# ouguangjun/Leg-KILO

Measured on NVIDIA H100. Metric: LiDAR point-iterations/sec through the ESKF point-to-plane update, higher is better.
Workload: dtype f64

## Files before the change

leg-kilo_b200/csrc/lk_api.cu:

```cuda
#include <cmath>
#include <cstdio>
#include <chrono>
#include <cstring>
#include <mutex>
#include <string>
#include <vector>

#include "lk_host.h"
#include "lk_kernels.h"
#include "lk_mapdev.h"

namespace lk {
int decode_pointcloud2_device(const uint8_t* h_data, uint32_t n, const lk_pc2_layout& L, float blind, int filter_num,
                              double time_scale, float* h_pts_out, float* h_intensity_out, uint32_t* n_out, cudaStream_t s,
                              std::string& err);
int preprocess_scan_device(const float* h_pts_in, uint32_t n, float leaf, float* h_pts_out, uint32_t* n_out,
                           uint32_t* h_bucket_offsets, float* h_bucket_curv, uint32_t* n_buckets, cudaStream_t s,
                           std::string& err);
size_t leg_kinematics_scratch_bytes(uint32_t n);
int leg_kinematics_device(const lk_leg_cfg& cfg, const lk_leg_state* h_in, uint32_t n, int redundancy,
                          lk_leg_track* track, lk_kinimu_meas* h_out, uint32_t* n_out, void* scratch, cudaStream_t s,
                          std::string& err);
}

// ... 24 lines not shown
          initsL(chunksL + align256(n_chunksL * sizeof(ChunkDesc))),
          bytes(initsL + align256(n_initsL * sizeof(StepInit))) {}
};

struct OutBlock {
    size_t x = 0, P = 0, clk = 0, n_eff = 0, status = 0, bytes = 0;
    OutBlock() = default;
    explicit OutBlock(int batch)
        : P(align256((size_t)batch * sizeof(lk_state))),
          clk(P + align256((size_t)batch * 900 * 8)),
          n_eff(clk + align256((size_t)batch * sizeof(lk_stream_clock))),
          status(n_eff + align256((size_t)batch * 4)),
          bytes(status + 256) {}
};

}

struct lk_context {
    int device = 0;
    cudaStream_t stream = nullptr;
    std::string err;
    lk_eskf_cfg ec;
    lk_map_cfg mc;
    Globals g;

    MapDevHost map;
    double last_slide_position[3] = {0.0, 0.0, 0.0};

    int batch = 0;
    uint64_t total_pts = 0;
    uint32_t total_chunks = 0, n_steps = 0, max_chunk_pts = 0;
    std::vector<ChunkDesc> h_chunks, h_chunksL;
    InBlock in;
    OutBlock out;
    DevBuf pts, world, sc, step, partial, ticket, fb_list, fb_cnt;
    DevBuf small_in, small_out, fx, fP, fQ, fclk;
    PinnedBuf h_small_in, h_small_out;
    DevView chunks, stepinit, x_in, P_in, clk_in, Q, x, P, clk, n_eff, status;
    DevBuf dbg_ok, dbg_h, dbg_z, dbg_R, dbg_key, tmp, trace, bar;
    DevBuf ins_pts, ins_root, ins_pend, ins_touched, ins_counters, ins_list;
    uint64_t ins_pend_nodes = 0;
    DevBuf mi_pts, mi_small, mi_ipts, mi_root, mi_touched, mi_counters, mi_list;
    PinnedBuf h_mi;
    int trace_on = 0;
    uint32_t trace_seq = 0;
    int lane_cache = 1;
    int use_fused = 1;
    FusedInline inl;
    DevBuf ll;
    uint32_t ll_epoch = 1;
    bool prev_fused = false;
    uint32_t fused_launches = 0, fused_launches_since_check = 0;
    int direct_io = 1, inline_in = 1, coop_launch = 0, pdl = 1, n_sms = 132, slim_p = 1;
    int fast_insert = 1;
    int fused_insert = 0;
    int debug_records = 0;
    bool direct = false, direct_ran = false, inline_ok = false;
    const float4* direct_pts = nullptr;
    float4* direct_world = nullptr;
    double hprof[8] = {0, 0, 0, 0, 0, 0, 0, 0};
    DevBuf Qc;
    DevBuf leg_scratch;
    std::vector<double> Q_shadow;

    cudaEvent_t ev0 = nullptr, ev1 = nullptr;
    std::vector<cudaEvent_t> kev;
    float last_total_ms = 0, last_residual_ms = 0;
    uint32_t last_launches = 0, last_residual_launches = 0;
    uint32_t acc_launches = 0, acc_residual_launches = 0;
    size_t nev = 0;
    int kernel_timing = 1;
    std::vector<StepInit> h_inits;
    std::vector<uint32_t> h_scan_pts;
    std::vector<uint32_t> h_scan_chunks;
    std::vector<StepInit> h_initsL;
    DevView chunksL, stepinitL;
    uint32_t total_chunksL = 0;

    ~lk_context() {
        for (cudaEvent_t e : kev) cudaEventDestroy(e);
        if (ev0) cudaEventDestroy(ev0);
        if (ev1) cudaEventDestroy(ev1);
        if (stream) cudaStreamDestroy(stream);
    }
};

namespace {

int fail(lk_handle h, int code, const std::string& msg) {
    if (h) h->err = msg;
    else g_create_error = msg;
    return code;
}

struct FusedGate {
    std::mutex m;
    cudaStream_t last = nullptr;
    cudaEvent_t ev = nullptr;
};
FusedGate& fused_gate(int device) {
    static FusedGate gates[64];
    return gates[(device >= 0 && device < 64) ? device : 0];
}

void enter(lk_handle h) {
    cudaSetDevice(h->device);
// ... 181 lines not shown
int lk_init_process_cov(const lk_eskf_cfg* c, double* Q) {
    if (!c || !Q) return LK_ERR_INVALID_ARG;
    for (int i = 0; i < 900; ++i) Q[i] = 0.0;
    const double d[7] = {c->vel_process_cov,     c->acc_bias_process_cov, c->gyr_bias_process_cov, c->imu_acc_process_cov,
                         c->imu_gyr_process_cov, c->kin_bias_process_cov, c->contact_process_cov};
    const int at[7] = {6, 9, 12, 18, 21, 24, 27};
    for (int b = 0; b < 7; ++b)
        for (int k = 0; k < 3; ++k) Q[(at[b] + k) * 30 + at[b] + k] = d[b];
    return LK_OK;
}

int lk_state_default(lk_state* x) {
    if (!x) return LK_ERR_INVALID_ARG;
    std::memset(x, 0, sizeof(*x));
    x->rot[0] = x->rot[4] = x->rot[8] = 1.0;
    x->grav[2] = -9.81;
    return LK_OK;
}

int lk_leg_track_default(lk_leg_track* t) {
    if (!t) return LK_ERR_INVALID_ARG;
    for (int k = 0; k < 4; ++k) t->in_contact[k] = 1;
    t->last_acc_z = 0.0f;
    t->last_gyr_z = 0.0f;
    return LK_OK;
}

int lk_host_alloc(void** p, size_t bytes) {
    if (!p) return LK_ERR_INVALID_ARG;
    cudaError_t e = cudaHostAlloc(p, bytes, cudaHostAllocDefault);
    if (e != cudaSuccess) {
        cudaGetLastError();
        return LK_ERR_OUT_OF_MEMORY;
    }
    return LK_OK;
}

int lk_host_free(void* p) {
    if (p) cudaFreeHost(p);
    return LK_OK;
}

int lk_set_param(lk_handle h, const char* name, double value) {
    if (!h || !name) return LK_ERR_INVALID_ARG;
    using IntKnob = int lk_context::*;
    static const struct {
        const char* name;
        IntKnob knob;
    } knobs[] = {{"kernel_timing", &lk_context::kernel_timing}, {"fused", &lk_context::use_fused},
                 {"lane_cache", &lk_context::lane_cache},       {"fast_insert", &lk_context::fast_insert},
                 {"fused_insert", &lk_context::fused_insert},   {"coop_launch", &lk_context::coop_launch},
                 {"pdl", &lk_context::pdl},                     {"slim_p", &lk_context::slim_p},
                 {"direct_io", &lk_context::direct_io},         {"inline_in", &lk_context::inline_in},
                 {"debug_records", &lk_context::debug_records}};
    for (const auto& k : knobs)
        if (!std::strcmp(name, k.name)) {
            h->*k.knob = (int)value;
            return LK_OK;
        }
    if (!std::strcmp(name, "trace")) {
        h->trace_on = (int)value;
        if (h->trace_on) {
            enter(h);
            LK_CUDA(h->err, h->trace.ensure((size_t)(1 << 16) * 8 * 8));
            LK_CUDA(h->err, cudaMemset(h->trace.p, 0, (size_t)(1 << 16) * 8 * 8));
        }
        h->trace_seq = 0;
        return LK_OK;
    }
    return fail(h, LK_ERR_INVALID_ARG, std::string("unknown parameter ") + name);
}

int lk_debug_read(lk_handle h, int what, void* dst, size_t bytes) {
    if (!h || !dst) return LK_ERR_INVALID_ARG;
    if (what == 3) {
        std::memcpy(dst, h->hprof, std::min(bytes, sizeof(h->hprof)));
        std::memset(h->hprof, 0, sizeof(h->hprof));
        return LK_OK;
    }
    enter(h);
    DevBuf* b = what == 0 ? &h->partial : (what == 1 ? &h->sc : &h->trace);
    if (what == 2) h->trace_seq = 0;
    if (bytes > b->cap) bytes = b->cap;
    LK_CUDA(h->err, cudaMemcpy(dst, b->p, bytes, cudaMemcpyDeviceToHost));
    return LK_OK;
}

int lk_sync(lk_handle h) {
    if (!h) return LK_ERR_INVALID_ARG;
    enter(h);
    LK_CUDA(h->err, cudaStreamSynchronize(h->stream));
    return check_stall(h);
}


int lk_map_reserve(lk_handle h, uint64_t max_roots, uint64_t max_nodes, uint64_t max_points) {
    if (!h) return LK_ERR_INVALID_ARG;
    h->map.reserve_roots = max_roots;
    h->map.reserve_nodes = max_nodes;
    h->map.reserve_points = max_points;
    return LK_OK;
}

int lk_map_upload(lk_handle h, const void* blob, size_t bytes) {
    if (!h || !blob) return fail(h, LK_ERR_INVALID_ARG, "null argument");
    enter(h);
    return map_upload_blob(h->map, h->g, blob, bytes, h->stream, h->err);
// ... 289 lines not shown
    LK_CUDA(h->err, cudaGetLastError());
    {
        const int rc = check_stall(h);
        if (rc) return rc;
    }
    LK_CUDA(h->err, cudaEventElapsedTime(&h->last_total_ms, h->ev0, h->ev1));
    float rms = 0;
    for (size_t i = 0; i + 1 < h->nev; i += 2) {
        float ms = 0;
        cudaEventElapsedTime(&ms, h->kev[i], h->kev[i + 1]);
        rms += ms;
    }
    h->last_residual_ms = rms;
    h->last_launches = h->acc_launches;
    h->last_residual_launches = h->acc_residual_launches;
    if (total_ms) *total_ms = h->last_total_ms;
    if (residual_kernel_ms) *residual_kernel_ms = rms;
    if (n_kernel_launches) *n_kernel_launches = h->last_launches;
    if (n_residual_launches) *n_residual_launches = h->last_residual_launches;
    return LK_OK;
}

namespace {
struct MeasQueue {
    const lk_imu_meas* d_imu = nullptr;
    const lk_kinimu_meas* d_kin = nullptr;
    const double* stamps = nullptr;
    uint32_t n = 0;
    double gravity = 9.81, acc_norm = 1.0;
};
}

static FusedArgs fused_args(lk_handle h, uint32_t first, int iters, bool insert, const MeasQueue* mq) {
    FusedArgs fa;
    std::memset(&fa, 0, sizeof(fa));
    fa.pts = h->direct ? h->direct_pts : h->pts.as<float4>();
    fa.world = h->direct ? h->direct_world : h->world.as<float4>();
    fa.inits = h->stepinit.as<StepInit>();
    fa.batch = h->batch;
    fa.n_steps = h->n_steps;
    fa.scan = first;
    fa.x_in = h->x_in.as<double>();
    fa.P_in = h->P_in.as<double>();
    fa.clk_in = h->clk_in.as<lk_stream_clock>();
    fa.Q = h->Q.as<double>();
    fa.x = h->x.as<double>();
    fa.P = h->P.as<double>();
    fa.clk = h->clk.as<lk_stream_clock>();
    fa.n_eff = h->n_eff.as<uint32_t>();
    fa.status = h->status.as<uint32_t>();
    fa.ll.chunk_rows = h->ll.as<ulonglong2>();
    fa.ll.group_rows = h->ll.as<ulonglong2>() + (size_t)2 * LL_MAX_CHUNKS * LL_ROW;
    fa.ll.stall = reinterpret_cast<uint32_t*>((char*)h->ll.p + LL_ROWS_BYTES);
    fa.epoch = h->ll_epoch;
    fa.iters = iters;
    fa.lane_cache = h->lane_cache;
    {
        const lk_stream_clock* ck = reinterpret_cast<const lk_stream_clock*>((const char*)h->h_small_in.p + h->in.clk) + first;
        const StepInit& in0 = h->h_inits[first];
        fa.slim_p = h->slim_p && h->n_steps == 1 && !mq && in0.active && in0.t_bucket == ck->last_predict_time &&
                    in0.t_bucket == ck->last_update_time;
    }
    const MapDev md = h->map.dev();
    fa.mv.slots = md.slots;
    fa.mv.hash_mask = md.hash_mask;
    fa.mv.nodes = md.nodes;
    fa.mv.hot = md.hot;
    if (mq) {
        fa.imu = mq->d_imu;
        fa.kin = mq->d_kin;
        fa.n_meas = mq->n;
        fa.gravity = mq->gravity;
        fa.acc_norm = mq->acc_norm;
    }
    fa.ecfg = h->ec;
    fa.trace = h->trace_on ? h->trace.as<unsigned long long>() + (size_t)(h->trace_seq++ % TRACE_AREAS) * TRACE_AREA : nullptr;
    fa.g = h->g;
    if (insert) {
        fa.insert = 1;
        fa.md = md;
        fa.ipts = reinterpret_cast<DevPoint*>(h->ins_pts.p);
        fa.iroot = h->ins_root.as<int>();
        fa.pend = h->ins_pend.as<int>();
        fa.touched = h->ins_touched.as<uint32_t>();
        fa.ins_counters = h->ins_counters.as<uint32_t>() + 2;
    }
    return fa;
}

static int run_fused(lk_handle h, uint32_t first, int iters, bool insert, const MeasQueue* mq, bool timed) {
    cudaStream_t s = h->stream;
    const uint32_t grid = insert ? (uint32_t)fused_max_blocks(h->device) : h->h_scan_chunks[first];
    FusedInline* inl = nullptr;
    if (h->inline_ok) {
        const char* hs = (const char*)h->h_small_in.p;
        inl = &h->inl;
        std::memcpy(inl->x, hs + h->in.x, sizeof(inl->x));
        std::memcpy(inl->P, hs + h->in.P, sizeof(inl->P));
        std::memcpy(inl->clk, hs + h->in.clk, sizeof(inl->clk));
        std::memcpy(inl->steps, h->h_inits.data(), h->h_inits.size() * sizeof(StepInit));
    }
    const uint32_t need = h->n_steps * ((uint32_t)iters + 2u) + 1u;
    if (h->ll_epoch > 0xE0000000u || need > 0x10000000u) {
        if (need > 0x10000000u) return fail(h, LK_ERR_INVALID_ARG, "steps x iters too large for one launch");
        LK_CUDA(h->err, cudaMemsetAsync(h->ll.p, 0, LL_BYTES, s));
        h->ll_epoch = 1;
        h->prev_fused = false;
    }
    const FusedArgs fa = fused_args(h, first, iters, insert, mq);
    h->ll_epoch += need;
    if (insert) h->prev_fused = false;
    if (timed) { cudaEventRecord(kev_get(h, h->nev++), s); h->prev_fused = false; }
    const int mode = h->coop_launch ? FUSED_LAUNCH_COOPERATIVE : ((h->pdl && h->prev_fused) ? FUSED_LAUNCH_PDL : FUSED_LAUNCH_PLAIN);
    {
        FusedGate& gate = fused_gate(h->device);
        std::lock_guard<std::mutex> lock(gate.m);
        if (gate.last && gate.last != s) {
            if (!gate.ev) LK_CUDA(h->err, cudaEventCreateWithFlags(&gate.ev, cudaEventDisableTiming));
            LK_CUDA(h->err, cudaEventRecord(gate.ev, gate.last));
            LK_CUDA(h->err, cudaStreamWaitEvent(s, gate.ev, 0));
        }
        gate.last = s;
        LK_CUDA(h->err, launch_scan_fused(fa, inl, grid, s, mode));
    }
    h->prev_fused = true;
    ++h->fused_launches_since_check;
    if (timed) { cudaEventRecord(kev_get(h, h->nev++), s); h->prev_fused = false; }
    ++h->acc_launches;
    ++h->acc_residual_launches;
    h->direct_ran = h->direct;
    return LK_OK;
}

static int run_kernels(lk_handle h, uint32_t first, uint32_t count, int iters, bool update_map, const MeasQueue* mq,
                       bool timed) {
    cudaStream_t s = h->stream;
    const int batch = h->batch;
    const bool big = count >= 2 && !h->h_initsL.empty();
    const std::vector<StepInit>& tin = big ? h->h_initsL : h->h_inits;
    const ChunkDesc* d_chunks = big ? h->chunksL.as<ChunkDesc>() : h->chunks.as<ChunkDesc>();
    const StepInit* d_inits = big ? h->stepinitL.as<StepInit>() : h->stepinit.as<StepInit>();
    uint32_t small_parity = 0;
    uint32_t mi = 0;
    if (mq) {
        LK_CUDA(h->err, cudaMemcpyAsync(h->x.as<lk_state>() + first, h->x_in.as<lk_state>() + first, sizeof(lk_state), cudaMemcpyDeviceToDevice, s));
        LK_CUDA(h->err, cudaMemcpyAsync(h->P.as<double>() + (size_t)first * 900, h->P_in.as<double>() + (size_t)first * 900, 900 * 8, cudaMemcpyDeviceToDevice, s));
        LK_CUDA(h->err, cudaMemcpyAsync(h->clk.as<lk_stream_clock>() + first, h->clk_in.as<lk_stream_clock>() + first, sizeof(lk_stream_clock), cudaMemcpyDeviceToDevice, s));
        LK_CUDA(h->err, cudaMemsetAsync(h->n_eff.as<uint32_t>() + first, 0, 4, s));
    }
    for (uint32_t k = 0; k < h->n_steps; ++k) {
        const StepInit* hin = tin.data() + (size_t)k * batch;
        uint32_t c0 = hin[first].chunk_begin, c1 = hin[first + count - 1].chunk_end;
        uint32_t m_obs0 = mi, m_obs1 = mi;
        if (mq && hin[first].active) {
            while (m_obs1 < mq->n && mq->stamps[m_obs1] < hin[first].t_bucket) ++m_obs1;
            mi = m_obs1;
        }
        const PredictArgs pa = predict_args(h, d_inits + (size_t)k * batch, (k == 0 && !mq) ? 1 : 0, first, count);
        if (mq && count == 1 && hin[first].active)
            launch_obs_predict_prepare(pa, mq->d_imu ? mq->d_imu + m_obs0 : nullptr, mq->d_kin ? mq->d_kin + m_obs0 : nullptr,
                                       m_obs1 - m_obs0, h->ec, mq->gravity, mq->acc_norm, s);
        else
// ... 504 lines not shown
```

leg-kilo_b200/csrc/lk_fused.cu:

```cuda
#include "lk_insert.cuh"
#include "lk_kernels.h"
#include "lk_obs.cuh"
#include "lk_pass.cuh"
#include "lk_predict.cuh"
#include "lk_solve.cuh"

namespace lk {

namespace {

#define FT(slot) do { if (a.trace && threadIdx.x == 0 && (slot) < 32) a.trace[(size_t)blockIdx.x * 32 + (slot)] = gtime(); } while (0)
#define FTI(slot) do { if (it_global < 3) FT(slot); } while (0)
#define FTS(slot) do { if (a.trace && blockIdx.x == 0 && threadIdx.x == 0 && k < 64) a.trace[(size_t)gridDim.x * 32 + (size_t)k * 8 + (slot)] = gtime(); } while (0)
#ifndef LK_HOP_TRACE
#define LK_HOP_TRACE 0
#endif
#define FT_HOPS() ((LK_HOP_TRACE && a.trace && it_global < 3) \
                       ? a.trace + (size_t)gridDim.x * 32 + 64 * 8 + (size_t)blockIdx.x * 16 + it_global * LL_HOP_SLOTS : nullptr)

constexpr int BLOCK = FB;
constexpr int WARPS = BLOCK / 32;

struct PredictScratch {
    double F[900];
// ... 30 lines not shown
    for (uint32_t t = blockIdx.x * (uint32_t)WARPS + (uint32_t)warp; t < n_touched; t += gridDim.x * (uint32_t)WARPS)
        warp_insert_root_scan(md, si->g, wt, __ldcg(&touched[t]), iroot, ipts, n_bucket, pend, lane);
}

static_assert(sizeof(PredictScratch) <= sizeof(((PassSmem<BLOCK, true>*)0)->tile) &&
                  sizeof(PredictScratch) <= sizeof(((PassSmem<BLOCK, false>*)0)->tile),
              "predict scratch must not reach the mbarriers");
static_assert(sizeof(FusedSmemIns) <= 227 * 1024, "one block per SM");
static_assert(sizeof(FusedSmem) + 1024 <= 132 * 1024, "the batch-of-one kernel's stack frames must fit in L1");

int carveout_percent(size_t smem, int dev) {
    int per_sm = 0, per_block = 0;
    cudaDeviceGetAttribute(&per_sm, cudaDevAttrMaxSharedMemoryPerMultiprocessor, dev);
    cudaDeviceGetAttribute(&per_block, cudaDevAttrReservedSharedMemoryPerBlock, dev);
    if (per_sm <= 0) return 100;
    const size_t need = smem + (size_t)per_block;
    const int pct = (int)((need * 100 + (size_t)per_sm - 1) / (size_t)per_sm);
    return pct < 100 ? pct : 100;
}

template <class SM>
__device__ __noinline__ void fused_predict(SM* sm, const double* Q, double dtc, double dt) {
    if (dtc != 0.0) {
        build_F(sm->u.pr.F, sm->f.x, dtc);
        cov_predict(sm->f.P, sm->u.pr.F, sm->u.pr.T, sm->u.pr.Ps, Q, dtc);
    }
    if (dt != 0.0) {
        if (threadIdx.x == 0) state_predict(sm->f.x, dt);
    }
    fence_proxy_async();
    __syncthreads();
}

template <class SM>
__device__ __noinline__ void fused_drain_queue(SM* sm, const FusedArgs& a, uint32_t& mi, double t_bucket) {
    bool drained = false;
    while (mi < a.n_meas) {
        const double ts = a.imu ? a.imu[mi].stamp : a.kin[mi].stamp;
        if (!(ts < t_bucket)) break;
        block_predict_to(&sm->f, sm->clk, ts, sm->u.pr.F, sm->u.pr.T, sm->u.pr.Ps, a.Q);
        if (a.imu) block_obs_imu<BLOCK>(&sm->f, &sm->u.pr.obs, a.imu + mi, &a.ecfg, a.gravity, a.acc_norm);
        else block_obs_kinimu<BLOCK>(&sm->f, &sm->u.pr.obs, a.kin + mi, &a.ecfg, a.gravity, a.acc_norm);
        if (threadIdx.x == 0) sm->clk[1] = ts;
        __syncthreads();
        ++mi;
        drained = true;
    }
    if (drained) {
        fence_proxy_async();
        __syncthreads();
    }
}

template <bool INL> struct InlineSel { typedef FusedInline type; };
template <> struct InlineSel<false> { typedef FusedNoInline type; };

__device__ __forceinline__ void grid_sync(const FusedArgs& a, uint32_t& sync_idx) {
    __threadfence();
    __syncthreads();
    if (threadIdx.x < 32) (void)ll_allreduce(a.ll, sync_idx & 1u, a.epoch + sync_idx, blockIdx.x, gridDim.x, 0.0, (int)threadIdx.x);
    ++sync_idx;
    __syncthreads();
    __threadfence();
    fence_proxy_async_global();
}

template <bool OBS, bool INL, bool INS>
__global__ void __launch_bounds__(BLOCK, 1) k_scan_fused(const __grid_constant__ FusedArgs a,
                                                         const __grid_constant__ typename InlineSel<INL>::type inl) {
    extern __shared__ __align__(16) unsigned char smem_raw[];
    FusedSmemT<!INS>* sm = reinterpret_cast<FusedSmemT<!INS>*>(smem_raw);
    const int tid = threadIdx.x, lane = tid & 31, warp = tid >> 5;
    const uint32_t scan = a.scan;
    asm volatile("griddepcontrol.launch_dependents;" ::: "memory");
    FT(0);
    {
        const double* Pin;
        const double* xin;
        const double* cin;
        if constexpr (INL) { Pin = inl.P; xin = inl.x; cin = inl.clk; }
        else { Pin = a.P_in + (size_t)scan * 900; xin = a.x_in + (size_t)scan * 36; cin = reinterpret_cast<const double*>(a.clk_in + scan); }
        if (a.slim_p && blockIdx.x != 0) {
            if (tid < 180) sm->f.P[(tid / 6) * 30 + tid % 6] = Pin[(tid / 6) * 30 + tid % 6];
        } else {
            for (int e = tid; e < 900; e += BLOCK) sm->f.P[e] = Pin[e];
        }
        if (tid < 36) sm->f.x[tid] = xin[tid];
        if (tid < 2) sm->clk[tid] = cin[tid];
    }
    if constexpr (INS) {
        FusedSmemIns* si = reinterpret_cast<FusedSmemIns*>(smem_raw);
        WarpTile* wt = si->wt + warp;
        if (lane == 0) {
            mbar_init(&wt->bar, 1);
            wt->phase = 0;
        }
        if (tid == 0) si->md = a.md;
        if (tid < (int)(sizeof(Globals) / 4)) reinterpret_cast<uint32_t*>(&si->g)[tid] = reinterpret_cast<const uint32_t*>(&a.g)[tid];
    }
    pass_init(&sm->u.pass);
    FT(1);
    uint32_t n_eff_total = 0;
    uint32_t phase = 0;
    uint32_t it_global = 0;
    uint32_t cslot = 0;
    uint32_t mi = 0;
    bool dep_waited = false;

    for (uint32_t k = 0; k < a.n_steps; ++k) {
        StepInit in;
        if constexpr (INL) in = inl.steps[k];
        else in = a.inits[(size_t)k * a.batch + scan];
        if (!in.active) continue;
        const uint32_t n_chunks = in.chunk_end - in.chunk_begin;
        const uint32_t my_start = in.pt_begin + blockIdx.x * (uint32_t)BLOCK;
        const uint32_t my_count = blockIdx.x < n_chunks ? min((uint32_t)BLOCK, in.pt_end - my_start) : 0u;
        float4 pre = make_float4(0.f, 0.f, 0.f, 0.f);
        if ((uint32_t)tid < my_count) pre = __ldg(a.pts + my_start + tid);
        FTS(0);
        if constexpr (OBS) fused_drain_queue(sm, a, mi, in.t_bucket);
        FTS(1);
        const double dtc = in.t_bucket - sm->clk[1];
        const double dt = in.t_bucket - sm->clk[0];
        if (dtc != 0.0 || dt != 0.0) fused_predict(sm, a.Q, dtc, dt);
        if (tid == 0) sm->clk[0] = in.t_bucket;
        FTS(2);
        bool updated = false, cov_pending = false;
        uint32_t n_last = 0;
        LaneCache lc;
        lc.have = 0;
        const bool more_steps = k + 1 < a.n_steps;
        for (int it = 0; it < a.iters; ++it, ++it_global) {
            scan_const_from(&sm->f, &sm->sc);
            __syncthreads();
            double acc[32];
#pragma unroll
            for (int i = 0; i < 32; ++i) acc[i] = 0.0;
            if (!a.lane_cache && lc.have == 2) lc.have = 1;
            points_pass<BLOCK, INS>(&sm->u.pass, phase, my_count, sm->sc, a.mv, a.g, lc, pre,
                                    [&](uint32_t, const Row& row) { accumulate_row(row, acc); });
            FTI(14 + it_global);
            const double tot = warp_transpose_sum(acc, lane);
            sm->slice[warp * 32 + lane] = tot;
            __syncthreads();
            FTI(2 + it_global * 4);
            if (it == 0) FTS(3);
            if (warp == 0) {
                double v = 0.0;
#pragma unroll
                for (int w = 0; w < WARPS; ++w) v += sm->slice[w * 32 + lane];
                if (!dep_waited) asm volatile("griddepcontrol.wait;" ::: "memory");
                sm->f.acc[lane] = ll_allreduce(a.ll, it_global & 1u, a.epoch + it_global, blockIdx.x, n_chunks, v, lane, FT_HOPS());
            }
            dep_waited = true;
            __syncthreads();
            FTI(3 + it_global * 4);
            if (it == 0) FTS(4);
            const bool last = it == a.iters - 1;
            const uint32_t n = block_solve_state(&sm->f);
            FTI(4 + it_global * 4);
            if (n > 0) {
                updated = true;
                if (tid == 0) sm->clk[1] = in.t_bucket;
                if (last) cov_pending = INS || more_steps || blockIdx.x == 0;
            }
            n_last = n;
        }
        n_eff_total += n_last;
        FTS(5);
        if constexpr (!INS) {
            if ((uint32_t)tid < my_count) {
                const double* X = sm->f.x;
                float4 o;
                o.x = (float)(X[0] * lc.pix + X[1] * lc.piy + X[2] * lc.piz + X[9]);
                o.y = (float)(X[3] * lc.pix + X[4] * lc.piy + X[5] * lc.piz + X[10]);
                o.z = (float)(X[6] * lc.pix + X[7] * lc.piy + X[8] * lc.piz + X[11]);
                o.w = updated ? 255.0f : 0.0f;
                a.world[my_start + tid] = o;
            }
            FT(20);
            if (cov_pending) block_cov_update<BLOCK>(&sm->f);
        } else {
            if (cov_pending) block_cov_update<BLOCK>(&sm->f);
            __syncthreads();
            scan_const_from(&sm->f, &sm->sc);
            __syncthreads();
            MapDev md = a.md;
            const uint32_t n_bucket = in.pt_end - in.pt_begin;
            if ((uint32_t)tid < my_count) {
                DevPoint p;
                make_insert_point(lc.pix, lc.piy, lc.piz, lc.pbx, lc.pby, lc.pbz, sm->sc, a.g, p);
                const uint32_t li = my_start + tid - in.pt_begin;
                a.ipts[li] = p;
                float4 o;
                o.x = (float)p.pw[0]; o.y = (float)p.pw[1]; o.z = (float)p.pw[2];
                o.w = updated ? 255.0f : 0.0f;
                a.world[my_start + tid] = o;
                a.iroot[li] = insert_register_point(md, a.g, p, a.pend, a.touched, &a.ins_counters[cslot]);
            }
            grid_sync(a, it_global);
            FTS(6);
            {
                const uint32_t n_touched = __ldcg(&a.ins_counters[cslot]);
                if (blockIdx.x == 0 && tid == 0) a.ins_counters[cslot ^ 1u] = 0;
                fused_insert_phase2(reinterpret_cast<FusedSmemIns*>(smem_raw), a.touched, a.iroot, a.ipts, a.pend, n_touched, n_bucket);
                cslot ^= 1u;
            }
            grid_sync(a, it_global);
            FTS(7);
        }
    }
    FT(30);
    if (blockIdx.x == 0) {
        if (!dep_waited) asm volatile("griddepcontrol.wait;" ::: "memory");
        __syncthreads();
        for (int e = tid; e < 900; e += BLOCK) a.P[(size_t)scan * 900 + e] = sm->f.P[e];
        if (tid < 36) a.x[(size_t)scan * 36 + tid] = sm->f.x[tid];
        if (tid < 2) reinterpret_cast<double*>(a.clk + scan)[tid] = sm->clk[tid];
        if (tid == 0) {
            a.n_eff[scan] = n_eff_total;
            *a.status = (*reinterpret_cast<volatile uint32_t*>(a.ll.stall) ? 1u : 0u) | (*reinterpret_cast<volatile uint32_t*>(&lk_stall_note[0]) ? 2u : 0u);
        }
    }
    FT(31);
}

template <bool OBS, bool INL, bool INS>
cudaError_t launch_one(const FusedArgs& a, const FusedInline* inl, uint32_t grid, cudaStream_t s, int mode) {
    auto kern = k_scan_fused<OBS, INL, INS>;
    constexpr size_t SMEM = INS ? sizeof(FusedSmemIns) : sizeof(FusedSmem);
    static PerDeviceOnce once;
    if (once.first()) {
        int dev = 0;
        cudaGetDevice(&dev);
        cudaError_t e = cudaFuncSetAttribute(kern, cudaFuncAttributeMaxDynamicSharedMemorySize, (int)SMEM);
        if (e != cudaSuccess) return e;
        e = cudaFuncSetAttribute(kern, cudaFuncAttributePreferredSharedMemoryCarveout, carveout_percent(SMEM, dev));
        if (e != cudaSuccess) return e;
    }
    typename InlineSel<INL>::type local_inl;
    const typename InlineSel<INL>::type* ip;
    if constexpr (INL) ip = inl;
    else { local_inl.unused = 0; ip = &local_inl; }
    if (mode == FUSED_LAUNCH_COOPERATIVE) {
        void* params[] = {(void*)&a, (void*)ip};
        return cudaLaunchCooperativeKernel((const void*)kern, dim3(grid), dim3(BLOCK), params, SMEM, s);
    }
    cudaLaunchConfig_t cfg = {};
    cfg.gridDim = dim3(grid);
    cfg.blockDim = dim3(BLOCK);
    cfg.dynamicSmemBytes = SMEM;
    cfg.stream = s;
    cudaLaunchAttribute at[1];
    at[0].id = cudaLaunchAttributeProgrammaticStreamSerialization;
    at[0].val.programmaticStreamSerializationAllowed = 1;
    cfg.attrs = at;
    cfg.numAttrs = mode == FUSED_LAUNCH_PDL ? 1 : 0;
    return cudaLaunchKernelEx(&cfg, kern, a, *ip);
}

}

size_t fused_smem_bytes() { return sizeof(FusedSmem); }

int fused_read_stall(uint32_t out[8]) {
    if (cudaMemcpyFromSymbol(out, lk_stall_note, 32) != cudaSuccess) return -1;
    if (out[0]) {
        const uint32_t z[8] = {0, 0, 0, 0, 0, 0, 0, 0};
        cudaMemcpyToSymbol(lk_stall_note, z, 32);
    }
    return 0;
}

int fused_max_blocks(int device) {
    static int cached[64];
// ... 21 lines not shown
```

leg-kilo_b200/csrc/lk_kernels.h:

```cpp
#pragma once
#include <cuda_runtime.h>

#include "lk_device.cuh"
#include "lk_llsync.cuh"
#include "lk_plane.cuh"

namespace lk {

struct StepInit {
    uint32_t chunk_begin, chunk_end;
    uint32_t pt_begin, pt_end;
    double t_bucket;
    uint32_t active;
    uint32_t pad;
};

struct ResidualArgs {
    const float4* pts;
    const HashSlot* slots;
    uint32_t hash_mask;
    const MapNode* nodes;
    const HotRec* hot;
    const ChunkDesc* chunks;
    uint32_t chunk_first;
// ... 47 lines not shown
void launch_predict_dt(double* x, double* P, const double* Q, const double* dt, int batch, int prop_state,
                       int prop_cov, cudaStream_t s);

struct ReprojectArgs {
    const float4* pts;
    float4* world;
    const ChunkDesc* chunks;
    uint32_t chunk_first;
    const ScanConst* sc;
    const ScanStep* step;
    Globals g;
};
void launch_reproject(const ReprojectArgs& a, uint32_t n_chunks, cudaStream_t s);


void launch_filter_obs(double* x, double* P, const double* Q, lk_stream_clock* clk, const lk_imu_meas* imu,
                       const lk_kinimu_meas* kin, uint32_t n, const lk_eskf_cfg& cfg, double gravity, double acc_norm,
                       cudaStream_t s);
void launch_update_by_points(double* x, double* P, uint32_t n, const double* h, const double* z, const double* r,
                             cudaStream_t s);

constexpr int FUSED_INLINE_STEPS = 64;
struct FusedInline {
    double x[36];
    double P[900];
    double clk[2];
    StepInit steps[FUSED_INLINE_STEPS];
};
struct FusedNoInline {
    int unused;
};

struct FusedArgs {
    const float4* pts;
    float4* world;
    const StepInit* inits;
    int batch;
    uint32_t n_steps;
    uint32_t scan;
    const double* x_in;
    const double* P_in;
    const lk_stream_clock* clk_in;
    const double* Q;
    double* x;
    double* P;
    lk_stream_clock* clk;
    uint32_t* n_eff;
    uint32_t* status;
    LLView ll;
    uint32_t epoch;
    int iters;
    int lane_cache;
    int slim_p;
    MapView mv;
    const lk_imu_meas* imu;
    const lk_kinimu_meas* kin;
    uint32_t n_meas;
    double gravity, acc_norm;
    lk_eskf_cfg ecfg;
    unsigned long long* trace;
    Globals g;
    int insert;
    MapDev md;
    DevPoint* ipts;
    int* iroot;
    int* pend;
    uint32_t* touched;
    uint32_t* ins_counters;
};
enum { FUSED_LAUNCH_PLAIN = 0, FUSED_LAUNCH_COOPERATIVE = 1, FUSED_LAUNCH_PDL = 2 };
size_t fused_smem_bytes();
int fused_max_blocks(int device);
int fused_read_stall(uint32_t out[8]);
cudaError_t launch_scan_fused(const FusedArgs& a, const FusedInline* inl, uint32_t grid, cudaStream_t s, int mode);

struct PerDeviceOnce {
    bool done[64] = {};
    bool first() {
        int d = 0;
        cudaGetDevice(&d);
        if (d < 0 || d >= 64) return true;
        if (done[d]) return false;
        done[d] = true;
        return true;
    }
};

}
```

leg-kilo_b200/csrc/lk_llsync.cuh:

```cuda
#pragma once
#include <cuda_runtime.h>
#include <stdint.h>

#include "lk_async.cuh"

namespace lk {

constexpr int LK_GROUP = 8;
constexpr int LL_ROW = 32;
constexpr int LL_MAX_CHUNKS = 160;
constexpr int LL_MAX_GROUPS = (LL_MAX_CHUNKS + LK_GROUP - 1) / LK_GROUP;
constexpr int LL_REPLICAS = 4;

struct LLView {
    ulonglong2* chunk_rows;
    ulonglong2* group_rows;
    uint32_t* stall;
};
constexpr size_t LL_ROWS_BYTES = (size_t)2 * (LL_MAX_CHUNKS + LL_REPLICAS * LL_MAX_GROUPS) * LL_ROW * sizeof(ulonglong2);
constexpr size_t LL_BYTES = LL_ROWS_BYTES + 64;
constexpr uint32_t LL_SPIN_LIMIT = 1u << 23;
constexpr int LL_HOP_SLOTS = 5;

__device__ __forceinline__ void ll_store(ulonglong2* p, double v, uint32_t tag) {
    const unsigned long long b = (unsigned long long)__double_as_longlong(v);
    const unsigned long long t = (unsigned long long)tag << 32;
    const unsigned long long w0 = (b & 0xffffffffull) | t, w1 = (b >> 32) | t;
    asm volatile("st.relaxed.gpu.global.v2.u64 [%0], {%1, %2};" ::"l"(p), "l"(w0), "l"(w1) : "memory");
}

__device__ __forceinline__ void ll_give_up(uint32_t* stall, uint32_t tag, uint32_t r0, uint32_t n, int lane) {
    if (atomicCAS(stall, 0u, 1u) == 0u) {
        stall[1] = blockIdx.x; stall[2] = tag; stall[3] = r0; stall[4] = n; stall[5] = (uint32_t)lane;
        __threadfence();
    }
}

template <int N, bool KEEP>
__device__ __forceinline__ double ll_sum_rows(const ulonglong2* rows, uint32_t r0, uint32_t n, uint32_t tag, int lane,
                                              uint32_t* stall, uint32_t& rounds, double first = 0.0, bool have_first = false) {
    static_assert(N <= 32, "one bit per row");
    const ulonglong2* p = rows + (size_t)r0 * LL_ROW + lane;
    unsigned long long w0[N], w1[N];
    const unsigned long long want = ((unsigned long long)tag << 32);
    uint32_t spins = 0;
    if constexpr (!KEEP) {
        bool all;
        do {
#pragma unroll
            for (int k = 0; k < N; ++k)
                if ((uint32_t)k < n && !(have_first && k == 0))
                    asm volatile("ld.relaxed.gpu.global.v2.u64 {%0, %1}, [%2];" : "=l"(w0[k]), "=l"(w1[k]) : "l"(p + (size_t)k * LL_ROW));
            all = true;
#pragma unroll
            for (int k = 0; k < N; ++k)
                if ((uint32_t)k < n && !(have_first && k == 0))
                    all = all && ((w0[k] & 0xffffffff00000000ull) == want) && ((w1[k] & 0xffffffff00000000ull) == want);
            ++spins;
            if (!all && ((spins & 0xfffu) == 0u)) {
                if (spins >= LL_SPIN_LIMIT || *reinterpret_cast<volatile uint32_t*>(stall) != 0u) {
                    ll_give_up(stall, tag, r0, n, lane);
                    break;
                }
            }
        } while (!all);
    } else {
        uint32_t todo = (n >= 32u ? 0xffffffffu : (1u << n) - 1u) & (have_first ? ~1u : ~0u);
        while (true) {
#pragma unroll
            for (int k = 0; k < N; ++k)
                if ((todo >> k) & 1u)
                    asm volatile("ld.relaxed.gpu.global.v2.u64 {%0, %1}, [%2];" : "=l"(w0[k]), "=l"(w1[k]) : "l"(p + (size_t)k * LL_ROW));
#pragma unroll
            for (int k = 0; k < N; ++k)
                if (((todo >> k) & 1u) && ((w0[k] & 0xffffffff00000000ull) == want) && ((w1[k] & 0xffffffff00000000ull) == want))
                    todo &= ~(1u << k);
            ++spins;
            if (todo == 0u) break;
            if ((spins & 0xfffu) == 0u) {
                if (spins >= LL_SPIN_LIMIT || *reinterpret_cast<volatile uint32_t*>(stall) != 0u) {
                    ll_give_up(stall, tag, r0, n, lane);
                    break;
                }
            }
        }
    }
    rounds = spins;
    double s = 0.0;
#pragma unroll
    for (int k = 0; k < N; ++k)
        if ((uint32_t)k < n) {
            const double v = (have_first && k == 0) ? first : __longlong_as_double((long long)((w0[k] & 0xffffffffull) | (w1[k] << 32)));
            s += v;
        }
    return s;
}

__device__ __forceinline__ double ll_allreduce(const LLView& ll, uint32_t parity, uint32_t tag, uint32_t b, uint32_t n_chunks,
                                               double v, int lane, unsigned long long* hops = nullptr) {
    constexpr size_t COPY = (size_t)LL_MAX_GROUPS * LL_ROW;
    ulonglong2* crows = ll.chunk_rows + (size_t)parity * LL_MAX_CHUNKS * LL_ROW;
    ulonglong2* grows = ll.group_rows + (size_t)parity * LL_REPLICAS * COPY;
    const uint32_t n_groups = (n_chunks + LK_GROUP - 1) / LK_GROUP;
    uint32_t r1 = 0, r2 = 0;
    if (b < n_chunks) {
        if ((b % LK_GROUP) == 0) {
            if (hops && lane == 0) hops[0] = gtime();
            const uint32_t n = min((uint32_t)LK_GROUP, n_chunks - b);
            const double s = ll_sum_rows<LK_GROUP, false>(crows, b, n, tag, lane, ll.stall, r1, v, true);
            if (hops && lane == 0) hops[1] = gtime();
            ulonglong2* g = grows + (size_t)(b / LK_GROUP) * LL_ROW + lane;
#pragma unroll
            for (int r = 0; r < LL_REPLICAS; ++r) ll_store(g + (size_t)r * COPY, s, tag);
            if (hops && lane == 0) hops[2] = gtime();
        } else {
            ll_store(crows + (size_t)b * LL_ROW + lane, v, tag);
            if (hops && lane == 0) hops[0] = gtime();
        }
    }
    const double t = ll_sum_rows<LL_MAX_GROUPS, true>(grows + (size_t)(b % LL_REPLICAS) * COPY, 0, n_groups, tag, lane, ll.stall, r2);
    if (hops) {
        r1 = __reduce_max_sync(0xffffffffu, r1);
        r2 = __reduce_max_sync(0xffffffffu, r2);
        if (lane == 0) {
            hops[3] = gtime();
            hops[4] = (unsigned long long)r1 | ((unsigned long long)r2 << 32);
        }
    }
    return t;
}

}
```

leg-kilo_b200/csrc/lk_solve.cuh:

```cuda
#pragma once
#include "lk_llsync.cuh"
#include "lk_point.cuh"

namespace lk {

struct BlockFilter {
    double x[36];
    double P[900];
    double acc[32];
    double A[36];
    double M[36];
    double y[6];
    double W[36];
    double delta[30];
    double Prow[180];
    double KH[180];
};

template <int NWARPS>
__device__ __forceinline__ void block_sum_partials(const double* partial, uint32_t c0, uint32_t c1, double* slice,
                                                   double* out) {
    const int tid = threadIdx.x, lane = tid & 31, warp = tid >> 5;
    const uint32_t n = c1 - c0, ng = (n + LK_GROUP - 1) / LK_GROUP;
    double tot = 0.0;
// ... 42 lines not shown
#pragma unroll
                for (int k = 0; k < 6; ++k) {
                    const int r = i < k ? i : k, c = i < k ? k : i;
                    ar[k] = f->acc[r * 6 - r * (r - 1) / 2 + (c - r)] * scale;
                }
                double m = (i == lane) ? 1.0 : 0.0;
#pragma unroll
                for (int k = 0; k < 6; ++k) m += ar[k] * Pc[k];
                double asel = ar[0];
#pragma unroll
                for (int t = 1; t < 6; ++t) asel = (lane - 7 == t) ? ar[t] : asel;
                const double bsel = f->acc[ACC_B + i] * scale;
                col[i] = lane < 6 ? m : (lane == 6 ? bsel : (lane < 13 ? asel : 0.0));
            }
            LK_SC(2);
            const bool okl = warp_solve6(col, lane);
            LK_SC(3);
            double y[6];
#pragma unroll
            for (int i = 0; i < 6; ++i) {
                y[i] = __shfl_sync(0xffffffffu, okl ? col[i] : 0.0, 6);
                if (lane >= 7 && lane < 13) f->W[i * 6 + (lane - 7)] = okl ? col[i] : 0.0;
            }
            double d = 0.0;
            if (lane < 30) {
#pragma unroll
                for (int k = 0; k < 6; ++k) d += f->P[lane * 30 + k] * y[k];
            }
            LK_SC(4);
            const double d0 = __shfl_sync(0xffffffffu, d, 0), d1 = __shfl_sync(0xffffffffu, d, 1),
                         d2 = __shfl_sync(0xffffffffu, d, 2);
            double rv = 0.0;
            if (lane < 9) {
                double E[9];
                so3_exp3(d0, d1, d2, E);
                const int i = lane / 3, j = lane % 3;
                const double e0 = j == 0 ? E[0] : (j == 1 ? E[1] : E[2]);
                const double e1 = j == 0 ? E[3] : (j == 1 ? E[4] : E[5]);
                const double e2 = j == 0 ? E[6] : (j == 1 ? E[7] : E[8]);
                rv = f->x[i * 3] * e0 + f->x[i * 3 + 1] * e1 + f->x[i * 3 + 2] * e2;
            }
            __syncwarp();
            if (lane < 9) f->x[lane] = rv;
            if (lane >= 3 && lane < 30) f->x[6 + lane] += d;
            LK_SC(5);
        }
        __syncthreads();
        LK_SC(6);
    }
#undef LK_SC
    return (uint32_t)(cnt + 0.5);
}

template <int NTHREADS>
__device__ __forceinline__ void block_cov_update(BlockFilter* f) {
    const int tid = threadIdx.x;
    for (int e = tid; e < 180; e += NTHREADS) {
        f->Prow[e] = f->P[e];
        int i = e / 6, j = e % 6;
        double s = 0.0;
#pragma unroll
        for (int k = 0; k < 6; ++k) s += f->P[i * 30 + k] * f->W[k * 6 + j];
        f->KH[e] = s;
    }
    __syncthreads();
    for (int e = tid; e < 900; e += NTHREADS) {
        int i = e / 30, j = e % 30;
        double s = 0.0;
#pragma unroll
        for (int k = 0; k < 6; ++k) s += f->KH[i * 6 + k] * f->Prow[k * 30 + j];
        f->P[e] -= s;
    }
    __syncthreads();
}

template <int NTHREADS>
__device__ __forceinline__ uint32_t block_solve_update(BlockFilter* f, bool last_iter, unsigned long long* clk = nullptr) {
    const uint32_t n = block_solve_state(f, clk);
    if (n > 0 && last_iter) block_cov_update<NTHREADS>(f);
    return n;
}

__device__ __forceinline__ void scan_const_from(const BlockFilter* f, ScanConst* sc) {
    const int tid = threadIdx.x;
    if (tid < 9) sc->R[tid] = f->x[tid];
    else if (tid < 12) sc->p[tid - 9] = f->x[tid];
    else if (tid < 24) {
        const int q = (tid - 12) % 6, o = (tid < 18) ? 0 : 3;
        const int i = (q < 3 ? 0 : (q < 5 ? 1 : 2)) + o, j = (q < 3 ? q : (q < 5 ? q - 2 : 2)) + o;
        const double v = 0.5 * (f->P[i * 30 + j] + f->P[j * 30 + i]);
        if (tid < 18) sc->Pth[q] = v; else sc->Ppp[q] = v;
    }
}

}
```

Baseline: 2.823 billion.

## Add finisher blocks that complete the last ESKF iteration off the chunk blocks

Launches extra finisher blocks on idle SMs. On the last iteration, chunk blocks only publish their partial reduction rows and exit. The finishers sum those rows, solve the state update, then split among themselves the world-point transform, covariance update and state writeback. The aim is to take the final allreduce wait and the tail work off the critical path of the chunk blocks. In exchange it adds an ack protocol, an extra replica of the group rows, a point copy buffer for direct IO, and more spin-wait synchronisation that could stall.

```diff
diff --git a/leg-kilo_b200/csrc/lk_api.cu b/leg-kilo_b200/csrc/lk_api.cu
--- a/leg-kilo_b200/csrc/lk_api.cu
+++ b/leg-kilo_b200/csrc/lk_api.cu
@@ -100,6 +100,7 @@
     bool prev_fused = false;
     uint32_t fused_launches = 0, fused_launches_since_check = 0;
     int direct_io = 1, inline_in = 1, coop_launch = 0, pdl = 1, n_sms = 132, slim_p = 1;
+    int finishers = 1;
     int fast_insert = 1;
     int fused_insert = 0;
     int debug_records = 0;
@@ -387,7 +388,7 @@
                  {"fused_insert", &lk_context::fused_insert},   {"coop_launch", &lk_context::coop_launch},
                  {"pdl", &lk_context::pdl},                     {"slim_p", &lk_context::slim_p},
                  {"direct_io", &lk_context::direct_io},         {"inline_in", &lk_context::inline_in},
-                 {"debug_records", &lk_context::debug_records}};
+                 {"debug_records", &lk_context::debug_records}, {"finishers", &lk_context::finishers}};
     for (const auto& k : knobs)
         if (!std::strcmp(name, k.name)) {
             h->*k.knob = (int)value;
@@ -783,6 +784,7 @@
     fa.ll.chunk_rows = h->ll.as<ulonglong2>();
     fa.ll.group_rows = h->ll.as<ulonglong2>() + (size_t)2 * LL_MAX_CHUNKS * LL_ROW;
     fa.ll.stall = reinterpret_cast<uint32_t*>((char*)h->ll.p + LL_ROWS_BYTES);
+    fa.ll.acks = reinterpret_cast<uint32_t*>((char*)h->ll.p + LL_ROWS_BYTES + 64);
     fa.epoch = h->ll_epoch;
     fa.iters = iters;
     fa.lane_cache = h->lane_cache;
@@ -804,6 +806,15 @@
         fa.gravity = mq->gravity;
         fa.acc_norm = mq->acc_norm;
     }
+    {
+        const StepInit& in0 = h->h_inits[first];
+        const uint32_t sms = (uint32_t)fused_max_blocks(h->device), chunks = h->h_scan_chunks[first];
+        if (h->finishers && !insert && fa.n_meas == 0 && h->n_steps == 1 && in0.active && in0.chunk_end - in0.chunk_begin == chunks &&
+            chunks > 0 && iters >= 1 && chunks < sms) {
+            fa.finishers = std::min(sms - chunks, (uint32_t)LL_MAX_FINISHERS);
+            if (h->direct) fa.pts_copy = h->pts.as<float4>();
+        }
+    }
     fa.ecfg = h->ec;
     fa.trace = h->trace_on ? h->trace.as<unsigned long long>() + (size_t)(h->trace_seq++ % TRACE_AREAS) * TRACE_AREA : nullptr;
     fa.g = h->g;
@@ -821,7 +832,6 @@
 
 static int run_fused(lk_handle h, uint32_t first, int iters, bool insert, const MeasQueue* mq, bool timed) {
     cudaStream_t s = h->stream;
-    const uint32_t grid = insert ? (uint32_t)fused_max_blocks(h->device) : h->h_scan_chunks[first];
     FusedInline* inl = nullptr;
     if (h->inline_ok) {
         const char* hs = (const char*)h->h_small_in.p;
@@ -839,6 +849,7 @@
         h->prev_fused = false;
     }
     const FusedArgs fa = fused_args(h, first, iters, insert, mq);
+    const uint32_t grid = insert ? (uint32_t)fused_max_blocks(h->device) : h->h_scan_chunks[first] + fa.finishers;
     h->ll_epoch += need;
     if (insert) h->prev_fused = false;
     if (timed) { cudaEventRecord(kev_get(h, h->nev++), s); h->prev_fused = false; }
diff --git a/leg-kilo_b200/csrc/lk_fused.cu b/leg-kilo_b200/csrc/lk_fused.cu
--- a/leg-kilo_b200/csrc/lk_fused.cu
+++ b/leg-kilo_b200/csrc/lk_fused.cu
@@ -106,6 +106,70 @@
     }
 }
 
+__device__ __forceinline__ float4 world_out(const double* X, double pix, double piy, double piz, bool updated) {
+    float4 o;
+    o.x = (float)(X[0] * pix + X[1] * piy + X[2] * piz + X[9]);
+    o.y = (float)(X[3] * pix + X[4] * piy + X[5] * piz + X[10]);
+    o.z = (float)(X[6] * pix + X[7] * piy + X[8] * piz + X[11]);
+    o.w = updated ? 255.0f : 0.0f;
+    return o;
+}
+
+template <class SM>
+__device__ __forceinline__ void store_state(SM* sm, const FusedArgs& a, uint32_t n_eff) {
+    const int tid = threadIdx.x;
+    if (tid < 36) a.x[(size_t)a.scan * 36 + tid] = sm->f.x[tid];
+    if (tid < 2) reinterpret_cast<double*>(a.clk + a.scan)[tid] = sm->clk[tid];
+    if (tid == 0) {
+        a.n_eff[a.scan] = n_eff;
+        *a.status = (*reinterpret_cast<volatile uint32_t*>(a.ll.stall) ? 1u : 0u) | (*reinterpret_cast<volatile uint32_t*>(&lk_stall_note[0]) ? 2u : 0u);
+    }
+}
+
+template <class SM>
+__device__ __noinline__ void fused_finish(SM* sm, const FusedArgs& a, const StepInit& in, uint32_t n_chunks, uint32_t it_global,
+                                          bool updated, bool dep_waited) {
+    const int tid = threadIdx.x;
+    const uint32_t fi = blockIdx.x - n_chunks, nf = gridDim.x - n_chunks;
+    if (!dep_waited) asm volatile("griddepcontrol.wait;" ::: "memory");
+    ll_sum_chunk_rows<WARPS>(a.ll, it_global & 1u, a.epoch + it_global, n_chunks, sm->u.pr.F, sm->f.acc);
+    FTI(3 + it_global * 4);
+    const uint32_t n = block_solve_state(&sm->f);
+    FTI(4 + it_global * 4);
+    if (n > 0) {
+        updated = true;
+        if (tid == 0) sm->clk[1] = in.t_bucket;
+    }
+    const float4* pts = a.pts;
+    if (a.pts_copy) {
+        __threadfence();
+        pts = a.pts_copy;
+    }
+    constexpr int U = 8;
+    const uint32_t step = nf * BLOCK;
+    for (uint32_t i0 = in.pt_begin + fi * BLOCK + tid; i0 < in.pt_end; i0 += U * step) {
+        float4 q[U];
+#pragma unroll
+        for (int u = 0; u < U; ++u)
+            if (i0 + u * step < in.pt_end) q[u] = __ldcg(pts + i0 + u * step);
+#pragma unroll
+        for (int u = 0; u < U; ++u)
+            if (i0 + u * step < in.pt_end) {
+                PointCtx p;
+                imu_point(q[u], a.g, p);
+                a.world[i0 + u * step] = world_out(sm->f.x, p.pix, p.piy, p.piz, updated);
+            }
+    }
+    FT(20);
+    if (n > 0) cov_prep(&sm->f, BLOCK);
+    __syncthreads();
+    for (uint32_t e = fi * BLOCK + tid; e < 900; e += nf * BLOCK)
+        a.P[(size_t)a.scan * 900 + e] = n > 0 ? cov_entry(&sm->f, (int)e) : sm->f.P[e];
+    FT(21);
+    if (fi == 0) store_state(sm, a, n);
+    FT(22);
+}
+
 template <bool INL> struct InlineSel { typedef FusedInline type; };
 template <> struct InlineSel<false> { typedef FusedNoInline type; };
 
@@ -126,6 +190,7 @@
     FusedSmemT<!INS>* sm = reinterpret_cast<FusedSmemT<!INS>*>(smem_raw);
     const int tid = threadIdx.x, lane = tid & 31, warp = tid >> 5;
     const uint32_t scan = a.scan;
+    const bool finisher = blockIdx.x + a.finishers >= gridDim.x;
     asm volatile("griddepcontrol.launch_dependents;" ::: "memory");
     FT(0);
     {
@@ -134,7 +199,7 @@
         const double* cin;
         if constexpr (INL) { Pin = inl.P; xin = inl.x; cin = inl.clk; }
         else { Pin = a.P_in + (size_t)scan * 900; xin = a.x_in + (size_t)scan * 36; cin = reinterpret_cast<const double*>(a.clk_in + scan); }
-        if (a.slim_p && blockIdx.x != 0) {
+        if (a.slim_p && !finisher && (a.finishers || blockIdx.x != 0)) {
             if (tid < 180) sm->f.P[(tid / 6) * 30 + tid % 6] = Pin[(tid / 6) * 30 + tid % 6];
         } else {
             for (int e = tid; e < 900; e += BLOCK) sm->f.P[e] = Pin[e];
@@ -199,18 +264,43 @@
             __syncthreads();
             FTI(2 + it_global * 4);
             if (it == 0) FTS(3);
+            const bool last = it == a.iters - 1;
+            if (!OBS && !INS && a.finishers && last) {
+                if (finisher) {
+                    fused_finish(sm, a, in, n_chunks, it_global, updated, dep_waited);
+                } else {
+                    if (!dep_waited) asm volatile("griddepcontrol.wait;" ::: "memory");
+                    if (a.pts_copy) {
+                        if ((uint32_t)tid < my_count) a.pts_copy[my_start + tid] = pre;
+                        __threadfence();
+                        __syncthreads();
+                    }
+                    if (warp == 0) {
+                        double v = 0.0;
+#pragma unroll
+                        for (int w = 0; w < WARPS; ++w) v += sm->slice[w * 32 + lane];
+                        ll_publish_row(a.ll, it_global & 1u, a.epoch + it_global, blockIdx.x, v, lane);
+                    }
+                }
+                FT(31);
+                return;
+            }
             if (warp == 0) {
                 double v = 0.0;
 #pragma unroll
                 for (int w = 0; w < WARPS; ++w) v += sm->slice[w * 32 + lane];
-                if (!dep_waited) asm volatile("griddepcontrol.wait;" ::: "memory");
-                sm->f.acc[lane] = ll_allreduce(a.ll, it_global & 1u, a.epoch + it_global, blockIdx.x, n_chunks, v, lane, FT_HOPS());
+                if (!dep_waited) {
+                    FT(23);
+                    asm volatile("griddepcontrol.wait;" ::: "memory");
+                    FT(24);
+                }
+                sm->f.acc[lane] = ll_allreduce(a.ll, it_global & 1u, a.epoch + it_global, blockIdx.x, n_chunks, v, lane, FT_HOPS(),
+                                               a.finishers, it_global >= 2);
             }
             dep_waited = true;
             __syncthreads();
             FTI(3 + it_global * 4);
             if (it == 0) FTS(4);
-            const bool last = it == a.iters - 1;
             const uint32_t n = block_solve_state(&sm->f);
             FTI(4 + it_global * 4);
             if (n > 0) {
@@ -223,15 +313,7 @@
         n_eff_total += n_last;
         FTS(5);
         if constexpr (!INS) {
-            if ((uint32_t)tid < my_count) {
-                const double* X = sm->f.x;
-                float4 o;
-                o.x = (float)(X[0] * lc.pix + X[1] * lc.piy + X[2] * lc.piz + X[9]);
-                o.y = (float)(X[3] * lc.pix + X[4] * lc.piy + X[5] * lc.piz + X[10]);
-                o.z = (float)(X[6] * lc.pix + X[7] * lc.piy + X[8] * lc.piz + X[11]);
-                o.w = updated ? 255.0f : 0.0f;
-                a.world[my_start + tid] = o;
-            }
+            if ((uint32_t)tid < my_count) a.world[my_start + tid] = world_out(sm->f.x, lc.pix, lc.piy, lc.piz, updated);
             FT(20);
             if (cov_pending) block_cov_update<BLOCK>(&sm->f);
         } else {
@@ -269,12 +351,7 @@
         if (!dep_waited) asm volatile("griddepcontrol.wait;" ::: "memory");
         __syncthreads();
         for (int e = tid; e < 900; e += BLOCK) a.P[(size_t)scan * 900 + e] = sm->f.P[e];
-        if (tid < 36) a.x[(size_t)scan * 36 + tid] = sm->f.x[tid];
-        if (tid < 2) reinterpret_cast<double*>(a.clk + scan)[tid] = sm->clk[tid];
-        if (tid == 0) {
-            a.n_eff[scan] = n_eff_total;
-            *a.status = (*reinterpret_cast<volatile uint32_t*>(a.ll.stall) ? 1u : 0u) | (*reinterpret_cast<volatile uint32_t*>(&lk_stall_note[0]) ? 2u : 0u);
-        }
+        store_state(sm, a, n_eff_total);
     }
     FT(31);
 }
diff --git a/leg-kilo_b200/csrc/lk_kernels.h b/leg-kilo_b200/csrc/lk_kernels.h
--- a/leg-kilo_b200/csrc/lk_kernels.h
+++ b/leg-kilo_b200/csrc/lk_kernels.h
@@ -123,6 +123,8 @@
     int iters;
     int lane_cache;
     int slim_p;
+    uint32_t finishers;
+    float4* pts_copy;
     MapView mv;
     const lk_imu_meas* imu;
     const lk_kinimu_meas* kin;
diff --git a/leg-kilo_b200/csrc/lk_llsync.cuh b/leg-kilo_b200/csrc/lk_llsync.cuh
--- a/leg-kilo_b200/csrc/lk_llsync.cuh
+++ b/leg-kilo_b200/csrc/lk_llsync.cuh
@@ -11,14 +11,17 @@
 constexpr int LL_MAX_CHUNKS = 160;
 constexpr int LL_MAX_GROUPS = (LL_MAX_CHUNKS + LK_GROUP - 1) / LK_GROUP;
 constexpr int LL_REPLICAS = 4;
+constexpr int LL_COPIES = LL_REPLICAS + 1;
+constexpr int LL_MAX_FINISHERS = 24;
 
 struct LLView {
     ulonglong2* chunk_rows;
     ulonglong2* group_rows;
     uint32_t* stall;
+    uint32_t* acks;
 };
-constexpr size_t LL_ROWS_BYTES = (size_t)2 * (LL_MAX_CHUNKS + LL_REPLICAS * LL_MAX_GROUPS) * LL_ROW * sizeof(ulonglong2);
-constexpr size_t LL_BYTES = LL_ROWS_BYTES + 64;
+constexpr size_t LL_ROWS_BYTES = (size_t)2 * (LL_MAX_CHUNKS + LL_COPIES * LL_MAX_GROUPS) * LL_ROW * sizeof(ulonglong2);
+constexpr size_t LL_BYTES = LL_ROWS_BYTES + 64 + 2 * LL_MAX_FINISHERS * sizeof(uint32_t);
 constexpr uint32_t LL_SPIN_LIMIT = 1u << 23;
 constexpr int LL_HOP_SLOTS = 5;
 
@@ -96,11 +99,29 @@
     return s;
 }
 
+__device__ __forceinline__ void ll_wait_acks(const uint32_t* acks, uint32_t fin, uint32_t tag, int lane, uint32_t* stall) {
+    uint32_t spins = 0;
+    bool mine = (uint32_t)lane >= fin;
+    while (!__all_sync(0xffffffffu, mine)) {
+        if (!mine) {
+            uint32_t w;
+            asm volatile("ld.acquire.gpu.global.u32 %0, [%1];" : "=r"(w) : "l"(acks + lane) : "memory");
+            mine = w == tag;
+        }
+        if ((++spins & 0xfffu) == 0u && (spins >= LL_SPIN_LIMIT || *reinterpret_cast<volatile uint32_t*>(stall) != 0u)) {
+            ll_give_up(stall, tag, 0, fin, lane);
+            break;
+        }
+    }
+}
+
 __device__ __forceinline__ double ll_allreduce(const LLView& ll, uint32_t parity, uint32_t tag, uint32_t b, uint32_t n_chunks,
-                                               double v, int lane, unsigned long long* hops = nullptr) {
+                                               double v, int lane, unsigned long long* hops = nullptr, uint32_t fin = 0,
+                                               bool acks_due = false) {
     constexpr size_t COPY = (size_t)LL_MAX_GROUPS * LL_ROW;
     ulonglong2* crows = ll.chunk_rows + (size_t)parity * LL_MAX_CHUNKS * LL_ROW;
-    ulonglong2* grows = ll.group_rows + (size_t)parity * LL_REPLICAS * COPY;
+    ulonglong2* grows = ll.group_rows + (size_t)parity * LL_COPIES * COPY;
+    uint32_t* acks = ll.acks + (size_t)parity * LL_MAX_FINISHERS;
     const uint32_t n_groups = (n_chunks + LK_GROUP - 1) / LK_GROUP;
     uint32_t r1 = 0, r2 = 0;
     if (b < n_chunks) {
@@ -110,15 +131,23 @@
             const double s = ll_sum_rows<LK_GROUP, false>(crows, b, n, tag, lane, ll.stall, r1, v, true);
             if (hops && lane == 0) hops[1] = gtime();
             ulonglong2* g = grows + (size_t)(b / LK_GROUP) * LL_ROW + lane;
+            if (fin && acks_due) ll_wait_acks(acks, fin, tag - 2u, lane, ll.stall);
 #pragma unroll
             for (int r = 0; r < LL_REPLICAS; ++r) ll_store(g + (size_t)r * COPY, s, tag);
+            if (fin) ll_store(g + (size_t)LL_REPLICAS * COPY, s, tag);
             if (hops && lane == 0) hops[2] = gtime();
         } else {
             ll_store(crows + (size_t)b * LL_ROW + lane, v, tag);
             if (hops && lane == 0) hops[0] = gtime();
         }
     }
-    const double t = ll_sum_rows<LL_MAX_GROUPS, true>(grows + (size_t)(b % LL_REPLICAS) * COPY, 0, n_groups, tag, lane, ll.stall, r2);
+    const bool finisher = fin && b >= n_chunks;
+    const double t = ll_sum_rows<LL_MAX_GROUPS, true>(grows + (size_t)(finisher ? LL_REPLICAS : b % LL_REPLICAS) * COPY, 0, n_groups,
+                                                      tag, lane, ll.stall, r2);
+    if (finisher) {
+        __syncwarp();
+        if (lane == 0) asm volatile("st.release.gpu.global.u32 [%0], %1;" ::"l"(acks + (b - n_chunks)), "r"(tag) : "memory");
+    }
     if (hops) {
         r1 = __reduce_max_sync(0xffffffffu, r1);
         r2 = __reduce_max_sync(0xffffffffu, r2);
@@ -130,4 +159,28 @@
     return t;
 }
 
+__device__ __forceinline__ void ll_publish_row(const LLView& ll, uint32_t parity, uint32_t tag, uint32_t b, double v, int lane) {
+    ll_store(ll.chunk_rows + ((size_t)parity * LL_MAX_CHUNKS + b) * LL_ROW + lane, v, tag);
 }
+
+template <int NWARPS>
+__device__ __forceinline__ void ll_sum_chunk_rows(const LLView& ll, uint32_t parity, uint32_t tag, uint32_t n_chunks, double* gs,
+                                                  double* out) {
+    const int tid = threadIdx.x, lane = tid & 31, warp = tid >> 5;
+    const ulonglong2* crows = ll.chunk_rows + (size_t)parity * LL_MAX_CHUNKS * LL_ROW;
+    const uint32_t n_groups = (n_chunks + LK_GROUP - 1) / LK_GROUP;
+    for (uint32_t g = (uint32_t)warp; g < n_groups; g += NWARPS) {
+        uint32_t rounds;
+        gs[g * 32 + lane] = ll_sum_rows<LK_GROUP, false>(crows, g * LK_GROUP, min((uint32_t)LK_GROUP, n_chunks - g * LK_GROUP), tag,
+                                                         lane, ll.stall, rounds);
+    }
+    __syncthreads();
+    if (tid < 32) {
+        double t = 0.0;
+        for (uint32_t g = 0; g < n_groups; ++g) t += gs[g * 32 + tid];
+        out[tid] = t;
+    }
+    __syncthreads();
+}
+
+}
diff --git a/leg-kilo_b200/csrc/lk_solve.cuh b/leg-kilo_b200/csrc/lk_solve.cuh
--- a/leg-kilo_b200/csrc/lk_solve.cuh
+++ b/leg-kilo_b200/csrc/lk_solve.cuh
@@ -118,10 +118,8 @@
     return (uint32_t)(cnt + 0.5);
 }
 
-template <int NTHREADS>
-__device__ __forceinline__ void block_cov_update(BlockFilter* f) {
-    const int tid = threadIdx.x;
-    for (int e = tid; e < 180; e += NTHREADS) {
+__device__ __forceinline__ void cov_prep(BlockFilter* f, int nthreads) {
+    for (int e = threadIdx.x; e < 180; e += nthreads) {
         f->Prow[e] = f->P[e];
         int i = e / 6, j = e % 6;
         double s = 0.0;
@@ -129,14 +127,21 @@
         for (int k = 0; k < 6; ++k) s += f->P[i * 30 + k] * f->W[k * 6 + j];
         f->KH[e] = s;
     }
+}
+
+__device__ __forceinline__ double cov_entry(const BlockFilter* f, int e) {
+    int i = e / 30, j = e % 30;
+    double s = 0.0;
+#pragma unroll
+    for (int k = 0; k < 6; ++k) s += f->KH[i * 6 + k] * f->Prow[k * 30 + j];
+    return f->P[e] - s;
+}
+
+template <int NTHREADS>
+__device__ __forceinline__ void block_cov_update(BlockFilter* f) {
+    cov_prep(f, NTHREADS);
     __syncthreads();
-    for (int e = tid; e < 900; e += NTHREADS) {
-        int i = e / 30, j = e % 30;
-        double s = 0.0;
-#pragma unroll
-        for (int k = 0; k < 6; ++k) s += f->KH[i * 6 + k] * f->Prow[k * 30 + j];
-        f->P[e] -= s;
-    }
+    for (int e = threadIdx.x; e < 900; e += NTHREADS) f->P[e] = cov_entry(f, e);
     __syncthreads();
 }
 
```

Result: faster. 3.151 billion, median of 6 (+11.7%).
